# yu-changqian/TorchSeg

Hardware: AMD Instinct MI355X
Metric: training images/sec (1024x1024) BiSeNet-R18 (higher is better)
Workload: dtype bf16

## Files before the change

### torchseg_amd/csrc/clshead.hip

```cpp
#include "tsg_mfma.h"
#include "tsg_dispatch.h"

namespace tsg {

constexpr int CH_MAXN = 32;
constexpr int CH_MAXC = 256;

struct ChGeom { int64_t B, HW, P; int C, N; };

template <int KS>
__global__ __launch_bounds__(256) void cls_fwd_k(const bf16_t* __restrict__ x, const float* __restrict__ w,
                                                 const float* __restrict__ bias, bf16_t* __restrict__ z, ChGeom g) {
  const int lane = threadIdx.x & 63, half = lane >> 5, l31 = lane & 31;
  bf16x8 af[KS];
#pragma unroll
  for (int ks = 0; ks < KS; ++ks) {
    uint32_t pk[4] = {0u, 0u, 0u, 0u};
    if (l31 < g.N) {
      const float* wr = w + (int64_t)l31 * g.C + ks * 16 + half * 8;
      const float4 a = *reinterpret_cast<const float4*>(wr), b = *reinterpret_cast<const float4*>(wr + 4);
      pk[0] = pack2_bf16(a.x, a.y); pk[1] = pack2_bf16(a.z, a.w); pk[2] = pack2_bf16(b.x, b.y); pk[3] = pack2_bf16(b.z, b.w);
    }
    const uint4 v = make_uint4(pk[0], pk[1], pk[2], pk[3]);
    af[ks] = __builtin_bit_cast(bf16x8, v);
  }
  float bs[16];
#pragma unroll
  for (int r = 0; r < 16; ++r) {
    const int n = (r & 3) + 8 * (r >> 2) + 4 * half;
    bs[r] = (bias && n < g.N) ? bias[n] : 0.f;
  }
  const int64_t ngroups = (g.P + 31) / 32;
  const int64_t wid = (int64_t)blockIdx.x * 4 + (threadIdx.x >> 6), nw = (int64_t)gridDim.x * 4;
  for (int64_t grp = wid; grp < ngroups; grp += nw) {
    const int64_t p = grp * 32 + l31;
    const bool ok = p < g.P;
    const bf16_t* xr = x + (ok ? p : g.P - 1) * g.C + half * 8;
    uint4 bv[KS];
#pragma unroll
    for (int ks = 0; ks < KS; ++ks) bv[ks] = *reinterpret_cast<const uint4*>(xr + ks * 16);
    f32x16 acc;
#pragma unroll
    for (int r = 0; r < 16; ++r) acc[r] = bs[r];
#pragma unroll
    for (int ks = 0; ks < KS; ++ks)
      acc = __builtin_amdgcn_mfma_f32_32x32x16_bf16(af[ks], __builtin_bit_cast(bf16x8, bv[ks]), acc, 0, 0, 0);
    if (ok) {
      const int64_t b = p / g.HW, hw = p - b * g.HW;
      bf16_t* zb = z + b * g.N * g.HW + hw;
#pragma unroll
      for (int r = 0; r < 16; ++r) {
        const int n = (r & 3) + 8 * (r >> 2) + 4 * half;
        if (n < g.N) zb[(int64_t)n * g.HW] = f32_to_bf16(acc[r]);
      }
    }
  }
}

constexpr int CH_RUN = 8;

__device__ __forceinline__ float ch_px(uint2 v, int j) {
  const uint32_t word = j < 2 ? v.x : v.y;
  return (j & 1) ? __uint_as_float(word & 0xffff0000u) : __uint_as_float(word << 16);
}

template <int CT>
__global__ __launch_bounds__(256) void cls_dgrad_k(const bf16_t* __restrict__ dz, const float* __restrict__ w,
                                                   bf16_t* __restrict__ dx, ChGeom g) {
  const int lane = threadIdx.x & 63, half = lane >> 5, l31 = lane & 31;
  bf16x8 bw[CT][2];
#pragma unroll
  for (int ct = 0; ct < CT; ++ct)
#pragma unroll
    for (int ks = 0; ks < 2; ++ks) {
      float f[8];
#pragma unroll
      for (int e = 0; e < 8; ++e) {
        const int n = 16 * ks + 8 * half + e;
        f[e] = n < g.N ? w[(int64_t)n * g.C + ct * 32 + l31] : 0.f;
      }
      const uint4 v = make_uint4(pack2_bf16(f[0], f[1]), pack2_bf16(f[2], f[3]), pack2_bf16(f[4], f[5]), pack2_bf16(f[6], f[7]));
      bw[ct][ks] = __builtin_bit_cast(bf16x8, v);
    }
  const int64_t ngroups = (g.P + 31) / 32;
  const int64_t wid = (int64_t)blockIdx.x * 4 + (threadIdx.x >> 6), nw = (int64_t)gridDim.x * 4;
  const bool even = (lane & 1) == 0;
  for (int64_t grp = wid; grp < ngroups; grp += nw) {
    const int64_t p = grp * 32 + l31;
    const bool ok = p < g.P;
    const int64_t pc = ok ? p : g.P - 1, b = pc / g.HW, hw = pc - b * g.HW;
    const bf16_t* zb = dz + b * g.N * g.HW + hw;
    bf16x8 az[2];
#pragma unroll
    for (int ks = 0; ks < 2; ++ks) {
      uint32_t h[8];
#pragma unroll
      for (int e = 0; e < 8; ++e) {
        const int n = 16 * ks + 8 * half + e;
        h[e] = (ok && n < g.N) ? (uint32_t)zb[(int64_t)n * g.HW] : 0u;
      }
      const uint4 v = make_uint4(h[0] | (h[1] << 16), h[2] | (h[3] << 16), h[4] | (h[5] << 16), h[6] | (h[7] << 16));
      az[ks] = __builtin_bit_cast(bf16x8, v);
    }
#pragma unroll
    for (int ct = 0; ct < CT; ++ct) {
      f32x16 acc;
#pragma unroll
      for (int r = 0; r < 16; ++r) acc[r] = 0.f;
      acc = __builtin_amdgcn_mfma_f32_32x32x16_bf16(az[0], bw[ct][0], acc, 0, 0, 0);
      acc = __builtin_amdgcn_mfma_f32_32x32x16_bf16(az[1], bw[ct][1], acc, 0, 0, 0);
#pragma unroll
      for (int q = 0; q < 8; ++q) {
        const int ra = 2 * q, rb = 2 * q + 1;
        const float got = __shfl_xor(even ? acc[rb] : acc[ra], 1, 64);
        const int r = even ? ra : rb;
        const int64_t pr = grp * 32 + (r & 3) + 8 * (r >> 2) + 4 * half;
        const uint32_t word = even ? pack2_bf16(acc[ra], got) : pack2_bf16(got, acc[rb]);
        if (pr < g.P) *reinterpret_cast<uint32_t*>(dx + pr * g.C + ct * 32 + (l31 & ~1)) = word;
      }
    }
  }
}

template <int CT>
__global__ __launch_bounds__(256) void cls_wgrad_k(const bf16_t* __restrict__ dz, const bf16_t* __restrict__ x,
                                                   float* __restrict__ part, ChGeom g) {
  __shared__ float img[CT * 32 * 32];
  const int lane = threadIdx.x & 63, half = lane >> 5, l31 = lane & 31, wave = threadIdx.x >> 6;
  f32x16 acc[CT];
#pragma unroll
  for (int ct = 0; ct < CT; ++ct)
#pragma unroll
    for (int r = 0; r < 16; ++r) acc[ct][r] = 0.f;
  const int64_t nsteps = g.P / 16;
  const int64_t wid = (int64_t)blockIdx.x * 4 + wave, nw = (int64_t)gridDim.x * 4;
  for (int64_t st = wid; st < nsteps; st += nw) {
    const int64_t p0 = st * 16 + 8 * half, b = p0 / g.HW, hw = p0 - b * g.HW;
    uint4 av = make_uint4(0u, 0u, 0u, 0u);
    if (l31 < g.N) av = *reinterpret_cast<const uint4*>(dz + (b * g.N + l31) * g.HW + hw);
    const bf16_t* xr = x + p0 * g.C + l31;
#pragma unroll
    for (int ct = 0; ct < CT; ++ct) {
      uint32_t h[8];
#pragma unroll
      for (int e = 0; e < 8; ++e) h[e] = (uint32_t)xr[(int64_t)e * g.C + ct * 32];
      const uint4 bv = make_uint4(h[0] | (h[1] << 16), h[2] | (h[3] << 16), h[4] | (h[5] << 16), h[6] | (h[7] << 16));
      acc[ct] = __builtin_amdgcn_mfma_f32_32x32x16_bf16(__builtin_bit_cast(bf16x8, av), __builtin_bit_cast(bf16x8, bv), acc[ct], 0, 0, 0);
    }
  }
  for (int wv = 0; wv < 4; ++wv) {
    if (wave == wv) {
#pragma unroll
      for (int ct = 0; ct < CT; ++ct)
#pragma unroll
        for (int r = 0; r < 16; ++r) {
          float* q = img + (ct * 32 + (r & 3) + 8 * (r >> 2) + 4 * half) * 32 + l31;
          *q = (wv == 0 ? 0.f : *q) + acc[ct][r];
        }
    }
    __syncthreads();
  }
  for (int i = threadIdx.x; i < CT * 32 * 32; i += 256) {
    const int ct = i / 1024, n = (i / 32) % 32, c = i % 32;
    if (n < g.N) part[((int64_t)blockIdx.x * g.N + n) * g.C + ct * 32 + c] = img[i];
  }
}

__global__ __launch_bounds__(256) void cls_dbias_k(const bf16_t* __restrict__ dz, float* __restrict__ part_b, ChGeom g) {
  __shared__ float smr[2 * 4];
  const int n = blockIdx.x;
  const int64_t b = blockIdx.y;
  const bf16_t* zp = dz + (b * g.N + n) * g.HW;
  float a = 0.f, dummy = 0.f;
  for (int64_t i = (int64_t)threadIdx.x * CH_RUN; i < g.HW; i += 256 * CH_RUN) {
    const uint4 v = *reinterpret_cast<const uint4*>(zp + i);
    const uint2 lo = make_uint2(v.x, v.y), hi = make_uint2(v.z, v.w);
#pragma unroll
    for (int j = 0; j < 4; ++j) a += ch_px(lo, j) + ch_px(hi, j);
  }
  block_sum2(a, dummy, smr);
  if (threadIdx.x == 0) part_b[b * g.N + n] = a;
}

__global__ __launch_bounds__(256) void cls_wgrad_fold(const float* __restrict__ part, const float* __restrict__ part_b, int nblk,
                                                      int nblk_b, int64_t nw, int N, float* __restrict__ dw,
                                                      float* __restrict__ db) {
  __shared__ double sm[4][64];
  const int col = threadIdx.x & 63, grp = threadIdx.x >> 6;
  const int64_t i = (int64_t)blockIdx.x * 64 + col;
  const bool bias_blk = blockIdx.x == gridDim.x - 1;
  const float* src = bias_blk ? part_b : part;
  const int64_t n_out = bias_blk ? N : nw, idx = bias_blk ? col : i;
  const int nb = bias_blk ? nblk_b : nblk;
  const int per = (nb + 3) / 4, b0 = grp * per, b1 = b0 + per < nb ? b0 + per : nb;
  double t = 0.0;
  if (idx < n_out) {
    for (int b = b0; b < b1; b += 8) {
      float v[8];
#pragma unroll
      for (int u = 0; u < 8; ++u) v[u] = b + u < b1 ? src[(int64_t)(b + u) * n_out + idx] : 0.f;
#pragma unroll
      for (int u = 0; u < 8; ++u) t += (double)v[u];
    }
  }
  sm[grp][col] = t;
  __syncthreads();
  if (grp == 0 && idx < n_out) {
    const double tot = (sm[0][col] + sm[1][col]) + (sm[2][col] + sm[3][col]);
    if (bias_blk) { if (db) db[idx] = (float)tot; }
    else dw[idx] = (float)tot;
  }
}

static int ch_geom(ChGeom* g, int64_t B, int64_t HW, int C, int N) {
  if (B <= 0 || HW <= 0 || C <= 0 || N <= 0 || N > CH_MAXN || C > CH_MAXC || C % 32 || C > 256 || (C & (C - 1)) || HW % 16) return TSG_E_SHAPE;
  if (B * HW > 0x3fffffffffLL / C) return TSG_E_SHAPE;
  g->B = B; g->HW = HW; g->P = B * HW; g->C = C; g->N = N;
  return 0;
}

constexpr int CH_WBLOCKS = 256;

}

using namespace tsg;

extern "C" {

int tsg_cls_head_supported(int dtype, int Cin, int n_classes, int64_t HW) {
  ChGeom g;
  return dtype == TSG_BF16 && ch_geom(&g, 1, HW, Cin, n_classes) == 0;
}

int tsg_cls_head_fwd(const void* x, const float* w, const float* bias, void* z, int64_t B, int64_t HW, int Cin, int n_classes,
                     void* stream) {
  if (!x || !w || !z) return TSG_E_NULL;
  ChGeom g;
  int e = ch_geom(&g, B, HW, Cin, n_classes);
  if (e) return e;
  if (!aligned16(x) || !aligned16(w)) return TSG_E_ALIGN;
  const int64_t ngroups = (g.P + 31) / 32;
  int64_t blocks = (ngroups + 3) / 4;
  if (blocks > 2048) blocks = 2048;
  hipStream_t st = (hipStream_t)stream;
  return with_int<1, 2, 4, 8, 16>(Cin / 16, [&](auto ks) {
    hipLaunchKernelGGL((cls_fwd_k<ks()>), dim3((unsigned)blocks), dim3(256), 0, st, (const bf16_t*)x, w, bias, (bf16_t*)z, g);
    TSG_CHECK_LAUNCH();
    return 0;
  });
}

int tsg_cls_head_dgrad(const void* dz, const float* w, void* dx, int64_t B, int64_t HW, int Cin, int n_classes, void* stream) {
  if (!dz || !w || !dx) return TSG_E_NULL;
  ChGeom g;
  int e = ch_geom(&g, B, HW, Cin, n_classes);
  if (e) return e;
  if (!aligned16(dz) || !aligned16(dx)) return TSG_E_ALIGN;
  const int64_t ngroups = (g.P + 31) / 32;
  int64_t blocks = (ngroups + 3) / 4;
  if (blocks > 1024) blocks = 1024;
  hipStream_t st = (hipStream_t)stream;
  return with_int<1, 2, 4, 8>(Cin / 32, [&](auto ct) {
    hipLaunchKernelGGL((cls_dgrad_k<ct()>), dim3((unsigned)blocks), dim3(256), 0, st, (const bf16_t*)dz, w, (bf16_t*)dx, g);
    TSG_CHECK_LAUNCH();
    return 0;
  });
}

size_t tsg_cls_head_wgrad_ws_bytes(int64_t B, int Cin, int n_classes) {
  if (B <= 0 || Cin <= 0 || n_classes <= 0) return 0;
  return ((size_t)CH_WBLOCKS * n_classes * Cin + (size_t)B * n_classes) * sizeof(float);
}

int tsg_cls_head_wgrad(const void* dz, const void* x, float* dw, float* dbias, int64_t B, int64_t HW, int Cin, int n_classes,
                       void* ws, size_t ws_bytes, void* stream) {
  if (!dz || !x || !dw || !ws) return TSG_E_NULL;
  ChGeom g;
  int e = ch_geom(&g, B, HW, Cin, n_classes);
  if (e) return e;
  if (B > 65535 || ws_bytes < tsg_cls_head_wgrad_ws_bytes(B, Cin, n_classes)) return B > 65535 ? TSG_E_SHAPE : TSG_E_WS;
  if (!aligned16(dz) || !aligned16(x) || !aligned16(ws)) return TSG_E_ALIGN;
  int64_t blocks = (g.P / 16 + 3) / 4;
  if (blocks > CH_WBLOCKS) blocks = CH_WBLOCKS;
  float* part = (float*)ws;
  float* part_b = part + (size_t)CH_WBLOCKS * n_classes * Cin;
  hipStream_t st = (hipStream_t)stream;
  e = with_int<1, 2, 4, 8>(Cin / 32, [&](auto ct) {
    hipLaunchKernelGGL((cls_wgrad_k<ct()>), dim3((unsigned)blocks), dim3(256), 0, st, (const bf16_t*)dz, (const bf16_t*)x, part, g);
    TSG_CHECK_LAUNCH();
    return 0;
  });
  if (e) return e;
  if (dbias) {
    hipLaunchKernelGGL(cls_dbias_k, dim3((unsigned)n_classes, (unsigned)B), dim3(256), 0, st, (const bf16_t*)dz, part_b, g);
    TSG_CHECK_LAUNCH();
  }
  const int64_t nw = (int64_t)n_classes * Cin;
  hipLaunchKernelGGL(cls_wgrad_fold, dim3((unsigned)((nw + 63) / 64 + 1)), dim3(256), 0, st, part, part_b, (int)blocks, (int)B, nw,
                     n_classes, dw, dbias);
  TSG_CHECK_LAUNCH();
  return 0;
}

}
```

### torchseg_amd/csrc/upsample.hip

```cpp
#include "tsg_dispatch.h"
#include "tsg_resample.h"

namespace tsg {

constexpr int kT = 256;

template <typename T, int V> struct OutVec;
template <> struct OutVec<float, 4> : Vec<float> {};
template <> struct OutVec<bf16_t, 8> : Vec<bf16_t> {};
template <typename T> struct OutVec<T, 1> {
  float v[1];
  __device__ __forceinline__ void load(const T* p) { v[0] = ld1<T>(p); }
  __device__ __forceinline__ void store(T* p) const { st1<T>(p, v[0]); }
};

template <typename T> __device__ __forceinline__ float round_as(float v);
template <> __device__ __forceinline__ float round_as<float>(float v) { return v; }
template <> __device__ __forceinline__ float round_as<bf16_t>(float v) { return bf16_to_f32(f32_to_bf16(v)); }

enum { kAddNone = 0, kAddOut = 1, kAddSrc = 2 };

template <typename T, int V, int ADD, int RB>
__global__ __launch_bounds__(kT) void up_fwd(const T* __restrict__ x, const T* __restrict__ add,
                                             T* __restrict__ y, int64_t NC, int IH, int IW, int OH,
                                             int OW, float sy, float sx) {
  const int vpr = OW / V;
  const int bands = (OH + RB - 1) / RB;
  const int64_t total = NC * bands * (int64_t)vpr;
  for (int64_t i = (int64_t)blockIdx.x * kT + threadIdx.x; i < total; i += (int64_t)gridDim.x * kT) {
    const int vx = (int)(i % vpr);
    const int64_t t = i / vpr;
    const int band = (int)(t % bands);
    const int64_t nc = t / bands;
    int x0[V], x1[V];
    float lx[V];
#pragma unroll
    for (int j = 0; j < V; ++j) src_index(sx, vx * V + j, IW, x0[j], x1[j], lx[j]);
    const T* src = x + nc * IH * (int64_t)IW;
    const T* src2 = ADD == kAddSrc ? add + nc * IH * (int64_t)IW : nullptr;
    auto tap = [&](int64_t off) -> float {
      return ADD == kAddSrc ? round_as<T>(ld1<T>(src + off) + ld1<T>(src2 + off)) : ld1<T>(src + off);
    };
    float h0[V], h1[V];
    int cy0 = -1, cy1 = -1;
    const int oy_end = (band + 1) * RB < OH ? (band + 1) * RB : OH;
    for (int oy = band * RB; oy < oy_end; ++oy) {
      int y0, y1; float ly;
      src_index(sy, oy, IH, y0, y1, ly);
      if (y0 != cy0) {
        if (y0 == cy1) {
#pragma unroll
          for (int j = 0; j < V; ++j) h0[j] = h1[j];
        } else {
          const int64_t r = (int64_t)y0 * IW;
#pragma unroll
          for (int j = 0; j < V; ++j) h0[j] = (1.f - lx[j]) * tap(r + x0[j]) + lx[j] * tap(r + x1[j]);
        }
        cy0 = y0;
        cy1 = -1;
      }
      if (y1 != cy1) {
        if (y1 == cy0) {
#pragma unroll
          for (int j = 0; j < V; ++j) h1[j] = h0[j];
        } else {
          const int64_t r = (int64_t)y1 * IW;
#pragma unroll
          for (int j = 0; j < V; ++j) h1[j] = (1.f - lx[j]) * tap(r + x0[j]) + lx[j] * tap(r + x1[j]);
        }
        cy1 = y1;
      }
      const float hy = 1.f - ly;
      const int64_t ooff = (nc * OH + oy) * (int64_t)OW + (int64_t)vx * V;
      OutVec<T, V> o, a;
      if (ADD == kAddOut) a.load(add + ooff);
#pragma unroll
      for (int j = 0; j < V; ++j) {
        float v = hy * h0[j] + ly * h1[j];
        if (ADD == kAddOut) v += a.v[j];
        o.v[j] = v;
      }
      o.store(y + ooff);
    }
  }
}

template <typename T, int MAXF>
__global__ __launch_bounds__(kT) void up_bwd(const T* __restrict__ dy, T* __restrict__ dx,
                                             int64_t NC, int IH, int IW, int OH, int OW, float sy,
                                             float sx) {
  const int64_t total = NC * IH * (int64_t)IW;
  for (int64_t i = (int64_t)blockIdx.x * kT + threadIdx.x; i < total; i += (int64_t)gridDim.x * kT) {
    const int ix = (int)(i % IW);
    const int64_t row = i / IW;
    const int iy = (int)(row % IH);
    const int64_t nc = row / IH;
    int xlo, xhi, ylo, yhi;
    footprint(sx, ix, OW, xlo, xhi);
    footprint(sy, iy, OH, ylo, yhi);
    float acc = 0.f;
    const T* base = dy + nc * OH * (int64_t)OW;
    if (MAXF > 0) {
      float wx[MAXF > 0 ? MAXF : 1];
#pragma unroll
      for (int j = 0; j < MAXF; ++j) wx[j] = (xlo + j <= xhi) ? tap_weight(sx, xlo + j, IW, ix) : 0.f;
      for (int oy = ylo; oy <= yhi; ++oy) {
        const float wy = tap_weight(sy, oy, IH, iy);
        if (wy != 0.f) {
          const T* r = base + (int64_t)oy * OW + xlo;
          float racc = 0.f;
#pragma unroll
          for (int j = 0; j < MAXF; ++j)
            if (xlo + j <= xhi) racc += wx[j] * ld1<T>(r + j);
          acc += wy * racc;
        }
      }
    } else {
      for (int oy = ylo; oy <= yhi; ++oy) {
        const float wy = tap_weight(sy, oy, IH, iy);
        if (wy != 0.f) {
          const T* r = base + (int64_t)oy * OW;
          float racc = 0.f;
          for (int ox = xlo; ox <= xhi; ++ox) racc += tap_weight(sx, ox, IW, ix) * ld1<T>(r + ox);
          acc += wy * racc;
        }
      }
    }
    st1<T>(dx + i, acc);
  }
}

template <typename T, int V, int MAXF>
__global__ void up_bwd_tiled(const T* __restrict__ dy, T* __restrict__ dx, int IH, int IW, int OH,
                             int OW, int RB, float sy, float sx) {
  extern __shared__ __attribute__((aligned(16))) float vrow[];
  const int nthreads = blockDim.x;
  const int tid = threadIdx.x;
  const int vpr = OW / V;
  const int bands = (IH + RB - 1) / RB;
  const int band = blockIdx.x % bands;
  const int64_t nc = blockIdx.x / bands;
  const int r0 = band * RB;
  const int r1 = (r0 + RB < IH) ? r0 + RB : IH;
  const T* src = dy + nc * OH * (int64_t)OW;
  for (int i = tid; i < (r1 - r0) * OW; i += nthreads) vrow[i] = 0.f;
  __syncthreads();
  int oy_lo = 0, oy_hi = OH - 1;
  if (sy > 0.f) {
    const float inv = 1.f / sy;
    int l = (int)ceilf((float)(r0 - 1) * inv) - 1;
    int h = (int)floorf((float)r1 * inv) + 1;
    oy_lo = l < 0 ? 0 : l;
    oy_hi = h > OH - 1 ? OH - 1 : h;
  }
  if (tid < vpr) {
    float accA[V], accB[V];
#pragma unroll
    for (int j = 0; j < V; ++j) { accA[j] = 0.f; accB[j] = 0.f; }
    int cur = -2;
    auto flush = [&](int row, const float (&acc)[V]) {
      if (row >= r0 && row < r1) {
        float* d = vrow + (row - r0) * OW + tid * V;
#pragma unroll
        for (int j = 0; j < V; ++j) d[j] = acc[j];
      }
    };
    auto absorb = [&](int oy, const OutVec<T, V>& g) {
      int y0, y1; float ly;
      src_index(sy, oy, IH, y0, y1, ly);
      if (y0 < r0 - 1 || y0 > r1 - 1) return;
      if (y0 != cur) {
        if (cur >= 0) {
          flush(cur, accA);
          if (y0 == cur + 1) {
#pragma unroll
            for (int j = 0; j < V; ++j) { accA[j] = accB[j]; accB[j] = 0.f; }
          } else {
            flush(cur + 1, accB);
#pragma unroll
            for (int j = 0; j < V; ++j) { accA[j] = 0.f; accB[j] = 0.f; }
          }
        }
        cur = y0;
      }
      const float hy = 1.f - ly;
      if (y1 == y0) {
#pragma unroll
        for (int j = 0; j < V; ++j) accA[j] += hy * g.v[j] + ly * g.v[j];
      } else {
#pragma unroll
        for (int j = 0; j < V; ++j) { accA[j] += hy * g.v[j]; accB[j] += ly * g.v[j]; }
      }
    };
    constexpr int U = 8;
    int oy = oy_lo;
    for (; oy + U - 1 <= oy_hi; oy += U) {
      OutVec<T, V> g[U];
#pragma unroll
      for (int u = 0; u < U; ++u) g[u].load(src + (int64_t)(oy + u) * OW + tid * V);
#pragma unroll
      for (int u = 0; u < U; ++u) absorb(oy + u, g[u]);
    }
    for (; oy <= oy_hi; ++oy) {
      OutVec<T, V> g;
      g.load(src + (int64_t)oy * OW + tid * V);
      absorb(oy, g);
    }
    if (cur >= 0) { flush(cur, accA); flush(cur + 1, accB); }
  }
  __syncthreads();
  for (int ix = tid; ix < IW; ix += nthreads) {
    int xlo, xhi;
    footprint(sx, ix, OW, xlo, xhi);
    float wx[MAXF];
#pragma unroll
    for (int j = 0; j < MAXF; ++j) wx[j] = (xlo + j <= xhi) ? tap_weight(sx, xlo + j, IW, ix) : 0.f;
    for (int r = r0; r < r1; ++r) {
      const float* v = vrow + (r - r0) * OW + xlo;
      float acc = 0.f;
#pragma unroll
      for (int j = 0; j < MAXF; ++j)
        if (xlo + j <= xhi) acc += wx[j] * v[j];
      st1<T>(dx + (nc * IH + r) * (int64_t)IW + ix, acc);
    }
  }
}

template <typename T, int V, int ADD>
__global__ __launch_bounds__(kT) void up_fwd_nhwc(const T* __restrict__ x, const T* __restrict__ add,
                                                  T* __restrict__ y, int64_t N, int C, int IH, int IW,
                                                  int OH, int OW, float sy, float sx) {
  const int G = C / V;
  const int64_t total = N * OH * (int64_t)OW * G;
  for (int64_t i = (int64_t)blockIdx.x * kT + threadIdx.x; i < total; i += (int64_t)gridDim.x * kT) {
    const int g = (int)(i % G);
    int64_t t = i / G;
    const int ox = (int)(t % OW); t /= OW;
    const int oy = (int)(t % OH);
    const int64_t n = t / OH;
    int y0, y1, x0, x1; float ly, lx;
    src_index(sy, oy, IH, y0, y1, ly);
    src_index(sx, ox, IW, x0, x1, lx);
    const float hy = 1.f - ly, hx = 1.f - lx;
    const T* b = x + n * IH * (int64_t)IW * C + g * V;
    OutVec<T, V> p00, p01, p10, p11, o, a;
    p00.load(b + ((int64_t)y0 * IW + x0) * C);
    p01.load(b + ((int64_t)y0 * IW + x1) * C);
    p10.load(b + ((int64_t)y1 * IW + x0) * C);
    p11.load(b + ((int64_t)y1 * IW + x1) * C);
    if (ADD == kAddOut) a.load(add + i * V);
    if (ADD == kAddSrc) {
      const T* b2 = add + n * IH * (int64_t)IW * C + g * V;
      OutVec<T, V> q00, q01, q10, q11;
      q00.load(b2 + ((int64_t)y0 * IW + x0) * C);
      q01.load(b2 + ((int64_t)y0 * IW + x1) * C);
      q10.load(b2 + ((int64_t)y1 * IW + x0) * C);
      q11.load(b2 + ((int64_t)y1 * IW + x1) * C);
#pragma unroll
      for (int j = 0; j < V; ++j) {
        p00.v[j] = round_as<T>(p00.v[j] + q00.v[j]); p01.v[j] = round_as<T>(p01.v[j] + q01.v[j]);
        p10.v[j] = round_as<T>(p10.v[j] + q10.v[j]); p11.v[j] = round_as<T>(p11.v[j] + q11.v[j]);
      }
    }
#pragma unroll
    for (int j = 0; j < V; ++j) {
      float v = hy * (hx * p00.v[j] + lx * p01.v[j]) + ly * (hx * p10.v[j] + lx * p11.v[j]);
      if (ADD == kAddOut) v += a.v[j];
      o.v[j] = v;
    }
    o.store(y + i * V);
  }
}

template <typename T, int V>
__global__ __launch_bounds__(kT) void up_bwd_nhwc(const T* __restrict__ dy, T* __restrict__ dx,
                                                  int64_t N, int C, int IH, int IW, int OH, int OW,
                                                  float sy, float sx) {
  const int G = C / V;
  const int64_t total = N * IH * (int64_t)IW * G;
  for (int64_t i = (int64_t)blockIdx.x * kT + threadIdx.x; i < total; i += (int64_t)gridDim.x * kT) {
    const int g = (int)(i % G);
    int64_t t = i / G;
    const int ix = (int)(t % IW); t /= IW;
    const int iy = (int)(t % IH);
    const int64_t n = t / IH;
    int xlo, xhi, ylo, yhi;
    footprint(sx, ix, OW, xlo, xhi);
    footprint(sy, iy, OH, ylo, yhi);
    float acc[V];
#pragma unroll
    for (int j = 0; j < V; ++j) acc[j] = 0.f;
    const T* b = dy + n * OH * (int64_t)OW * C + g * V;
    for (int oy = ylo; oy <= yhi; ++oy) {
      const float wy = tap_weight(sy, oy, IH, iy);
      if (wy == 0.f) continue;
      for (int ox = xlo; ox <= xhi; ++ox) {
        const float w = wy * tap_weight(sx, ox, IW, ix);
        if (w != 0.f) {
          OutVec<T, V> p;
          p.load(b + ((int64_t)oy * OW + ox) * C);
#pragma unroll
          for (int j = 0; j < V; ++j) acc[j] += w * p.v[j];
        }
      }
    }
    OutVec<T, V> o;
#pragma unroll
    for (int j = 0; j < V; ++j) o.v[j] = acc[j];
    o.store(dx + i * V);
  }
}

template <typename T, int V>
__global__ __launch_bounds__(256) void up_bwd_nhwc_split(const T* __restrict__ dy, T* __restrict__ dx, int64_t N, int C,
                                                         int IH, int IW, int OH, int OW, float sy, float sx, int gpb) {
  __shared__ float red[256 * V];
  const int G = C / V, RS = 256 / gpb;
  const int tid = threadIdx.x, gl = tid % gpb, rs = tid / gpb;
  const int g = blockIdx.y * gpb + gl;
  int64_t t = blockIdx.x;
  const int ix = (int)(t % IW); t /= IW;
  const int iy = (int)(t % IH);
  const int64_t n = t / IH;
  int xlo, xhi, ylo, yhi;
  footprint(sx, ix, OW, xlo, xhi);
  footprint(sy, iy, OH, ylo, yhi);
  float acc[V];
#pragma unroll
  for (int j = 0; j < V; ++j) acc[j] = 0.f;
  if (rs < RS && g < G) {
    const T* b = dy + n * OH * (int64_t)OW * C + g * V;
    for (int oy = ylo + rs; oy <= yhi; oy += RS) {
      const float wy = tap_weight(sy, oy, IH, iy);
      if (wy == 0.f) continue;
      for (int ox = xlo; ox <= xhi; ++ox) {
        const float w = wy * tap_weight(sx, ox, IW, ix);
        if (w != 0.f) {
          OutVec<T, V> p;
          p.load(b + ((int64_t)oy * OW + ox) * C);
#pragma unroll
          for (int j = 0; j < V; ++j) acc[j] += w * p.v[j];
        }
      }
    }
  }
#pragma unroll
  for (int j = 0; j < V; ++j) red[tid * V + j] = acc[j];
  __syncthreads();
  if (rs == 0 && g < G) {
    OutVec<T, V> o;
#pragma unroll
    for (int j = 0; j < V; ++j) {
      float s = 0.f;
      for (int q = 0; q < RS; ++q) s += red[(q * gpb + gl) * V + j];
      o.v[j] = s;
    }
    o.store(dx + (blockIdx.x * (int64_t)G + g) * V);
  }
}

template <int EB>
__global__ __launch_bounds__(kT) void nearest_fwd(const void* __restrict__ x, void* __restrict__ y,
                                                  int64_t NC, int IH, int IW, int OH, int OW,
                                                  float sy, float sx) {
  typedef typename std::conditional<EB == 1, uint8_t,
          typename std::conditional<EB == 2, uint16_t,
          typename std::conditional<EB == 4, uint32_t, uint64_t>::type>::type>::type E;
  const int64_t total = NC * OH * (int64_t)OW;
  for (int64_t i = (int64_t)blockIdx.x * kT + threadIdx.x; i < total; i += (int64_t)gridDim.x * kT) {
    const int ox = (int)(i % OW);
    const int64_t row = i / OW;
    const int oy = (int)(row % OH);
    const int64_t nc = row / OH;
    int iy = (int)floorf((float)oy * sy); if (iy > IH - 1) iy = IH - 1;
    int ix = (int)floorf((float)ox * sx); if (ix > IW - 1) ix = IW - 1;
    ((E*)y)[i] = ((const E*)x)[(nc * IH + iy) * IW + ix];
  }
}

static int grid_for(int64_t work) {
  int64_t g = (work + kT - 1) / kT;
  if (g > 8192) g = 8192;
  if (g < 1) g = 1;
  return (int)g;
}

}

using namespace tsg;

template <typename T, bool ACC>
__global__ __launch_bounds__(kT) void resize_hp_k(const T* __restrict__ x, float* __restrict__ y, int64_t NC, int IH,
                                                  int IW, int OH, int OW) {
  const double sy = 1.0 / ((double)OH / (double)IH), sx = 1.0 / ((double)OW / (double)IW);
  const int64_t total = NC * OH * (int64_t)OW;
  for (int64_t i = (int64_t)blockIdx.x * kT + threadIdx.x; i < total; i += (int64_t)gridDim.x * kT) {
    const int ox = (int)(i % OW);
    const int64_t t = i / OW;
    const int oy = (int)(t % OH);
    const int64_t nc = t / OH;
    int y0, y1, x0, x1; float wy, wx;
    hp_index(oy, sy, IH, y0, y1, wy);
    hp_index(ox, sx, IW, x0, x1, wx);
    const T* p = x + nc * IH * (int64_t)IW;
    const float a = ld1<T>(p + (int64_t)y0 * IW + x0), b = ld1<T>(p + (int64_t)y0 * IW + x1);
    const float c = ld1<T>(p + (int64_t)y1 * IW + x0), d = ld1<T>(p + (int64_t)y1 * IW + x1);
    const float v = (1.f - wy) * ((1.f - wx) * a + wx * b) + wy * ((1.f - wx) * c + wx * d);
    y[i] = ACC ? y[i] + v : v;
  }
}

extern "C" {

static int up_fwd_launch(const void* x, const void* add, int add_mode, void* y, int dtype, int64_t NC,
                         int IH, int IW, int OH, int OW, void* stream) {
  if (!x || !y || (add_mode != kAddNone && !add)) return TSG_E_NULL;
  if (dtype != TSG_F32 && dtype != TSG_BF16) return TSG_E_DTYPE;
  if (NC <= 0 || IH <= 0 || IW <= 0 || OH <= 0 || OW <= 0) return TSG_E_SHAPE;
  hipStream_t st = (hipStream_t)stream;
  const float sy = ac_scale(IH, OH), sx = ac_scale(IW, OW);
  const int native = native_vec(dtype);
  const bool vec = (OW % native == 0) && aligned16(y) && (add_mode != kAddOut || aligned16(add));
  const int V = vec ? native : 1;
  const int grid = grid_for(NC * ((OH + 15) / 16) * (int64_t)(OW / V));
  return with_elem_vec(dtype, vec, [&](auto t, auto v) { return with_int<kAddOut, kAddSrc, kAddNone>(add_mode, [&](auto a) {
    typedef typename decltype(t)::type T;
    hipLaunchKernelGGL((up_fwd<T, v(), a(), 16>), dim3(grid), dim3(kT), 0, st, (const T*)x, (const T*)add, (T*)y, NC, IH, IW,
                       OH, OW, sy, sx);
    TSG_CHECK_LAUNCH();
    return 0;
  }); });
}

int tsg_upsample_bilinear_ac_fwd(const void* x, const void* add, void* y, int dtype, int64_t NC,
                                 int IH, int IW, int OH, int OW, void* stream) {
  return up_fwd_launch(x, add, add ? kAddOut : kAddNone, y, dtype, NC, IH, IW, OH, OW, stream);
}

int tsg_upsample_bilinear_ac_presum_fwd(const void* x, const void* x2, void* y, int dtype, int64_t NC,
                                        int IH, int IW, int OH, int OW, void* stream) {
  return up_fwd_launch(x, x2, kAddSrc, y, dtype, NC, IH, IW, OH, OW, stream);
}

int tsg_upsample_bilinear_ac_bwd(const void* dy, void* dx, int dtype, int64_t NC, int IH, int IW,
                                 int OH, int OW, void* stream) {
  if (!dy || !dx) return TSG_E_NULL;
  if (dtype != TSG_F32 && dtype != TSG_BF16) return TSG_E_DTYPE;
  if (NC <= 0 || IH <= 0 || IW <= 0 || OH <= 0 || OW <= 0) return TSG_E_SHAPE;
  hipStream_t st = (hipStream_t)stream;
  const float sy = ac_scale(IH, OH), sx = ac_scale(IW, OW);
  int need = sx > 0.f ? (int)floorf(2.f / sx) + 4 : OW;
  const int maxf = need <= 9 ? 9 : need <= 21 ? 21 : need <= 37 ? 37 : 0;
  const int native = native_vec(dtype);
  if (need <= 37 && OW % native == 0 && OW / native <= 1024 && OW >= IW && aligned16(dy)) {
    int threads = ((OW / native + 63) / 64) * 64;
    if (threads < 128) threads = 128;
    int RB = 8;
    while (RB > 1 && (size_t)RB * OW * sizeof(float) > 48 * 1024) RB >>= 1;
    if ((size_t)RB * OW * sizeof(float) <= 64 * 1024) {
      const int bands = (IH + RB - 1) / RB;
      const int64_t blocks = NC * bands;
      if (blocks <= 0x7fffffffLL) {
        const size_t sh = (size_t)RB * OW * sizeof(float);
        return with_elem(dtype, [&](auto t) { return with_int<9, 21, 37>(maxf, [&](auto f) {
          typedef typename decltype(t)::type T;
          hipLaunchKernelGGL((up_bwd_tiled<T, Vec<T>::N, f()>), dim3((unsigned)blocks), dim3(threads), sh, st, (const T*)dy,
                             (T*)dx, IH, IW, OH, OW, RB, sy, sx);
          TSG_CHECK_LAUNCH();
          return 0;
        }); });
      }
    }
  }
  const int grid = grid_for(NC * IH * (int64_t)IW);
  return with_elem(dtype, [&](auto t) { return with_int<9, 21, 37, 0>(maxf, [&](auto f) {
    typedef typename decltype(t)::type T;
    hipLaunchKernelGGL((up_bwd<T, f()>), dim3(grid), dim3(kT), 0, st, (const T*)dy, (T*)dx, NC, IH, IW, OH, OW, sy, sx);
    TSG_CHECK_LAUNCH();
    return 0;
  }); });
}

static int up_fwd_nhwc_launch(const void* x, const void* add, int add_mode, void* y, int dtype, int64_t N,
                              int C, int IH, int IW, int OH, int OW, void* stream) {
  if (!x || !y || (add_mode != kAddNone && !add)) return TSG_E_NULL;
  if (dtype != TSG_F32 && dtype != TSG_BF16) return TSG_E_DTYPE;
  const int V = native_vec(dtype);
  if (N <= 0 || C <= 0 || C % V || IH <= 0 || IW <= 0 || OH <= 0 || OW <= 0) return TSG_E_SHAPE;
  if (!aligned16(x) || !aligned16(y) || (add && !aligned16(add))) return TSG_E_ALIGN;
  hipStream_t st = (hipStream_t)stream;
  const float sy = ac_scale(IH, OH), sx = ac_scale(IW, OW);
  const int grid = grid_for(N * OH * (int64_t)OW * (C / V));
  return with_elem(dtype, [&](auto t) { return with_int<kAddOut, kAddSrc, kAddNone>(add_mode, [&](auto a) {
    typedef typename decltype(t)::type T;
    hipLaunchKernelGGL((up_fwd_nhwc<T, Vec<T>::N, a()>), dim3(grid), dim3(kT), 0, st, (const T*)x, (const T*)add, (T*)y, N, C,
                       IH, IW, OH, OW, sy, sx);
    TSG_CHECK_LAUNCH();
    return 0;
  }); });
}

int tsg_upsample_bilinear_ac_nhwc_fwd(const void* x, const void* add, void* y, int dtype, int64_t N,
                                      int C, int IH, int IW, int OH, int OW, void* stream) {
  return up_fwd_nhwc_launch(x, add, add ? kAddOut : kAddNone, y, dtype, N, C, IH, IW, OH, OW, stream);
}

int tsg_upsample_bilinear_ac_nhwc_presum_fwd(const void* x, const void* x2, void* y, int dtype, int64_t N,
                                             int C, int IH, int IW, int OH, int OW, void* stream) {
  return up_fwd_nhwc_launch(x, x2, kAddSrc, y, dtype, N, C, IH, IW, OH, OW, stream);
}

int tsg_upsample_bilinear_ac_nhwc_bwd(const void* dy, void* dx, int dtype, int64_t N, int C, int IH,
                                      int IW, int OH, int OW, void* stream) {
  if (!dy || !dx) return TSG_E_NULL;
  if (dtype != TSG_F32 && dtype != TSG_BF16) return TSG_E_DTYPE;
  const int V = native_vec(dtype);
  if (N <= 0 || C <= 0 || C % V || IH <= 0 || IW <= 0 || OH <= 0 || OW <= 0) return TSG_E_SHAPE;
  if (!aligned16(dy) || !aligned16(dx)) return TSG_E_ALIGN;
  hipStream_t st = (hipStream_t)stream;
  const float sy = ac_scale(IH, OH), sx = ac_scale(IW, OW);
  const int G = C / V;
  if (N * IH * (int64_t)IW * G < 65536 && OH >= 8 * IH && N * IH * (int64_t)IW <= 0x7fffffffLL) {
    int gpb = 256;
    while (gpb > G) gpb >>= 1;
    if (gpb < 1) gpb = 1;
    while (gpb > 8 && N * IH * (int64_t)IW * ((G + gpb - 1) / gpb) < 512) gpb >>= 1;
    const dim3 grid2((unsigned)(N * IH * IW), (unsigned)((G + gpb - 1) / gpb));
    return with_elem(dtype, [&](auto t) {
      typedef typename decltype(t)::type T;
      hipLaunchKernelGGL((up_bwd_nhwc_split<T, Vec<T>::N>), grid2, dim3(256), 0, st, (const T*)dy, (T*)dx, N, C, IH, IW, OH, OW,
                         sy, sx, gpb);
      TSG_CHECK_LAUNCH();
      return 0;
    });
  }
  const int grid = grid_for(N * IH * (int64_t)IW * (C / V));
  return with_elem(dtype, [&](auto t) {
    typedef typename decltype(t)::type T;
    hipLaunchKernelGGL((up_bwd_nhwc<T, Vec<T>::N>), dim3(grid), dim3(kT), 0, st, (const T*)dy, (T*)dx, N, C, IH, IW, OH, OW, sy, sx);
    TSG_CHECK_LAUNCH();
    return 0;
  });
}

int tsg_upsample_nearest_fwd(const void* x, void* y, int elem_bytes, int64_t NC, int IH, int IW,
                             int OH, int OW, void* stream) {
  if (!x || !y) return TSG_E_NULL;
  if (NC <= 0 || IH <= 0 || IW <= 0 || OH <= 0 || OW <= 0) return TSG_E_SHAPE;
  hipStream_t st = (hipStream_t)stream;
  const float sy = (float)IH / (float)OH, sx = (float)IW / (float)OW;
  const int grid = grid_for(NC * OH * (int64_t)OW);
#define GO(EB) hipLaunchKernelGGL((nearest_fwd<EB>), dim3(grid), dim3(kT), 0, st, x, y, NC, IH, IW, OH, OW, sy, sx)
  switch (elem_bytes) {
    case 1: GO(1); break;
    case 2: GO(2); break;
    case 4: GO(4); break;
    case 8: GO(8); break;
    default: return TSG_E_DTYPE;
  }
#undef GO
  TSG_CHECK_LAUNCH();
  return 0;
}

int tsg_resize_bilinear_hp(const void* x, float* y, int dtype, int64_t NC, int IH, int IW, int OH, int OW,
                           int accumulate, void* stream) {
  if (!x || !y) return TSG_E_NULL;
  if (dtype != TSG_F32 && dtype != TSG_BF16) return TSG_E_DTYPE;
  if (NC <= 0 || IH <= 0 || IW <= 0 || OH <= 0 || OW <= 0) return TSG_E_SHAPE;
  hipStream_t st = (hipStream_t)stream;
  const int grid = grid_for(NC * OH * (int64_t)OW);
  return with_elem(dtype, [&](auto t) { return with_flag(accumulate != 0, [&](auto acc) {
    typedef typename decltype(t)::type T;
    hipLaunchKernelGGL((resize_hp_k<T, acc()>), dim3(grid), dim3(kT), 0, st, (const T*)x, y, NC, IH, IW, OH, OW);
    TSG_CHECK_LAUNCH();
    return 0;
  }); });
}

}
```

Baseline: 1336.

## Add LDS-staged streaming class-head kernels and row-strip bilinear upsample

Result: no change. 1344 (median of 6 runs) (+0.6%).

```diff
diff --git a/torchseg_amd/csrc/clshead.hip b/torchseg_amd/csrc/clshead.hip
--- a/torchseg_amd/csrc/clshead.hip
+++ b/torchseg_amd/csrc/clshead.hip
@@ -53,6 +53,87 @@
         const int n = (r & 3) + 8 * (r >> 2) + 4 * half;
         if (n < g.N) zb[(int64_t)n * g.HW] = f32_to_bf16(acc[r]);
       }
+    }
+  }
+}
+
+typedef u32x4 __attribute__((may_alias)) lds_u32x4;
+__device__ __forceinline__ void wave_lds_sync() {
+  __builtin_amdgcn_fence(__ATOMIC_RELEASE, "wavefront");
+  __builtin_amdgcn_wave_barrier();
+  __builtin_amdgcn_fence(__ATOMIC_ACQUIRE, "wavefront");
+}
+__device__ __forceinline__ u32x4 zero_u32x4() { const u32x4 z = {0u, 0u, 0u, 0u}; return z; }
+
+template <int KS>
+__global__ __launch_bounds__(KS == 16 ? 128 : 256) void cls_fwd_stream_k(const bf16_t* __restrict__ x,
+                                                                         const float* __restrict__ w,
+                                                                         const float* __restrict__ bias,
+                                                                         bf16_t* __restrict__ z, ChGeom g) {
+  constexpr int W = KS == 16 ? 2 : 4;
+  constexpr int C = KS * 16, ROW = C / 8 + 1;
+  __shared__ uint4 tile[W * 32 * ROW];
+  const int lane = threadIdx.x & 63, half = lane >> 5, l31 = lane & 31, wave = threadIdx.x >> 6;
+  uint4* my = tile + wave * 32 * ROW;
+  bf16x8 af[KS];
+#pragma unroll
+  for (int ks = 0; ks < KS; ++ks) {
+    uint32_t pk[4] = {0u, 0u, 0u, 0u};
+    if (l31 < g.N) {
+      const float* wr = w + (int64_t)l31 * C + ks * 16 + half * 8;
+      const float4 a = *reinterpret_cast<const float4*>(wr), b = *reinterpret_cast<const float4*>(wr + 4);
+      pk[0] = pack2_bf16(a.x, a.y); pk[1] = pack2_bf16(a.z, a.w); pk[2] = pack2_bf16(b.x, b.y); pk[3] = pack2_bf16(b.z, b.w);
+    }
+    const uint4 v = make_uint4(pk[0], pk[1], pk[2], pk[3]);
+    af[ks] = __builtin_bit_cast(bf16x8, v);
+  }
+  float bs[16];
+#pragma unroll
+  for (int r = 0; r < 16; ++r) {
+    const int n = (r & 3) + 8 * (r >> 2) + 4 * half;
+    bs[r] = (bias && n < g.N) ? bias[n] : 0.f;
+  }
+  const int64_t ngroups = (g.P + 31) / 32;
+  const bool even = (lane & 1) == 0;
+  auto fetch = [&](int64_t grp, uint4 (&bv)[KS]) {
+    const int64_t left = (g.P - grp * 32) * (C / 8);
+    const uint4* src = reinterpret_cast<const uint4*>(x) + grp * 32 * (C / 8) + lane;
+#pragma unroll
+    for (int i = 0; i < KS; ++i) bv[i] = i * 64 + lane < left ? src[i * 64] : make_uint4(0u, 0u, 0u, 0u);
+  };
+  const int64_t wid = (int64_t)blockIdx.x * W + wave, nw = (int64_t)gridDim.x * W;
+  uint4 bv[KS];
+  if (wid < ngroups) fetch(wid, bv);
+  for (int64_t grp = wid; grp < ngroups; grp += nw) {
+#pragma unroll
+    for (int i = 0; i < KS; ++i) {
+      const int j = i * 64 + lane;
+      my[(j / (C / 8)) * ROW + j % (C / 8)] = bv[i];
+    }
+    wave_lds_sync();
+    if (grp + nw < ngroups) fetch(grp + nw, bv);
+    f32x16 acc;
+#pragma unroll
+    for (int r = 0; r < 16; ++r) acc[r] = bs[r];
+#pragma unroll
+    for (int ks = 0; ks < KS; ++ks) {
+      const uint4 fr = my[l31 * ROW + 2 * ks + half];
+      acc = __builtin_amdgcn_mfma_f32_32x32x16_bf16(af[ks], __builtin_bit_cast(bf16x8, fr), acc, 0, 0, 0);
+    }
+    wave_lds_sync();
+    const int64_t p = grp * 32 + (l31 & ~1);
+    const bool ok = p < g.P;
+    const int64_t pc = ok ? p : 0, b = pc / g.HW, hw = pc - b * g.HW;
+    bf16_t* zb = z + b * g.N * g.HW + hw;
+#pragma unroll
+    for (int q = 0; q < 8; ++q) {
+      const int ra = 2 * q, rb = 2 * q + 1;
+      const float got = __shfl_xor(even ? acc[rb] : acc[ra], 1, 64);
+      const int r = even ? ra : rb;
+      const int n = (r & 3) + 8 * (r >> 2) + 4 * half;
+      const uint32_t word = even ? ((uint32_t)f32_to_bf16(acc[ra]) | ((uint32_t)f32_to_bf16(got) << 16))
+                                 : ((uint32_t)f32_to_bf16(got) | ((uint32_t)f32_to_bf16(acc[rb]) << 16));
+      if (ok && n < g.N) *reinterpret_cast<uint32_t*>(zb + (int64_t)n * g.HW) = word;
     }
   }
 }
@@ -123,6 +204,92 @@
 }
 
 template <int CT>
+__global__ __launch_bounds__(256) void cls_dgrad_stream_k(const bf16_t* __restrict__ dz, const float* __restrict__ w,
+                                                          bf16_t* __restrict__ dx, ChGeom g) {
+  constexpr int CP = CT >= 2 ? 2 : 1;
+  constexpr int OROW = CP == 2 ? 192 : 64;
+  constexpr int WB = 2048 + 32 * OROW;
+  __shared__ __attribute__((aligned(16))) unsigned char lds[4 * WB];
+  const int lane = threadIdx.x & 63, half = lane >> 5, l31 = lane & 31, sub = (lane >> 4) & 1, i16 = lane & 15;
+  unsigned char* zt = lds + (threadIdx.x >> 6) * WB;
+  unsigned char* ot = zt + 2048;
+  const lds_v4i16* zfr = (const lds_v4i16*)(zt + (8 * half + (i16 >> 2)) * 64 + (16 * sub + 4 * (i16 & 3)) * 2);
+  bf16x8 bw[CT][2];
+#pragma unroll
+  for (int ct = 0; ct < CT; ++ct)
+#pragma unroll
+    for (int ks = 0; ks < 2; ++ks) {
+      float f[8];
+#pragma unroll
+      for (int e = 0; e < 8; ++e) {
+        const int n = 16 * ks + 8 * half + e;
+        f[e] = n < g.N ? w[(int64_t)n * g.C + ct * 32 + l31] : 0.f;
+      }
+      const uint4 v = make_uint4(pack2_bf16(f[0], f[1]), pack2_bf16(f[2], f[3]), pack2_bf16(f[4], f[5]), pack2_bf16(f[6], f[7]));
+      bw[ct][ks] = __builtin_bit_cast(bf16x8, v);
+    }
+  const int64_t ngroups = (g.P + 31) / 32;
+  const int64_t wid = (int64_t)blockIdx.x * 4 + (threadIdx.x >> 6), nw = (int64_t)gridDim.x * 4;
+  const bool even = (lane & 1) == 0;
+  auto fetch = [&](int64_t grp, u32x4 (&zv)[2]) {
+#pragma unroll
+    for (int i = 0; i < 2; ++i) {
+      const int q = lane + 64 * i, n = q >> 2;
+      const int64_t p0 = grp * 32 + 8 * (q & 3);
+      zv[i] = zero_u32x4();
+      if (n < g.N && p0 < g.P) {
+        const int64_t b = p0 / g.HW, hw = p0 - b * g.HW;
+        zv[i] = *reinterpret_cast<const u32x4*>(dz + (b * g.N + n) * g.HW + hw);
+      }
+    }
+  };
+  u32x4 zv[2];
+  if (wid < ngroups) fetch(wid, zv);
+  for (int64_t grp = wid; grp < ngroups; grp += nw) {
+#pragma unroll
+    for (int i = 0; i < 2; ++i) *reinterpret_cast<lds_u32x4*>(zt + (lane + 64 * i) * 16) = zv[i];
+    wave_lds_sync();
+    union { v4i16 q[2]; bf16x8 v; } az[2];
+#pragma unroll
+    for (int ks = 0; ks < 2; ++ks) {
+      az[ks].q[0] = __builtin_amdgcn_ds_read_tr16_b64_v4i16((lds_v4i16*)(zfr + ks * 128));
+      az[ks].q[1] = __builtin_amdgcn_ds_read_tr16_b64_v4i16((lds_v4i16*)(zfr + ks * 128 + 32));
+    }
+    if (grp + nw < ngroups) fetch(grp + nw, zv);
+#pragma unroll
+    for (int cp = 0; cp < CT / CP; ++cp) {
+#pragma unroll
+      for (int c2 = 0; c2 < CP; ++c2) {
+        const int ct = cp * CP + c2;
+        f32x16 acc;
+#pragma unroll
+        for (int r = 0; r < 16; ++r) acc[r] = 0.f;
+        acc = __builtin_amdgcn_mfma_f32_32x32x16_bf16(az[0].v, bw[ct][0], acc, 0, 0, 0);
+        acc = __builtin_amdgcn_mfma_f32_32x32x16_bf16(az[1].v, bw[ct][1], acc, 0, 0, 0);
+#pragma unroll
+        for (int q = 0; q < 8; ++q) {
+          const int ra = 2 * q, rb = 2 * q + 1;
+          const float got = __shfl_xor(even ? acc[rb] : acc[ra], 1, 64);
+          const int r = even ? ra : rb;
+          const int row = (r & 3) + 8 * (r >> 2) + 4 * half;
+          const uint32_t word = even ? pack2_bf16(acc[ra], got) : pack2_bf16(got, acc[rb]);
+          *reinterpret_cast<lds_u32*>(ot + row * OROW + (c2 * 32 + (l31 & ~1)) * 2) = word;
+        }
+      }
+      wave_lds_sync();
+#pragma unroll
+      for (int i = 0; i < 2 * CP; ++i) {
+        const int j = i * 64 + lane, px = j / (CP * 4), cc = j % (CP * 4);
+        const u32x4 v = *reinterpret_cast<const lds_u32x4*>(ot + px * OROW + cc * 16);
+        const int64_t pr = grp * 32 + px;
+        if (pr < g.P) *reinterpret_cast<u32x4*>(dx + pr * g.C + cp * CP * 32 + cc * 8) = v;
+      }
+      wave_lds_sync();
+    }
+  }
+}
+
+template <int CT>
 __global__ __launch_bounds__(256) void cls_wgrad_k(const bf16_t* __restrict__ dz, const bf16_t* __restrict__ x,
                                                    float* __restrict__ part, ChGeom g) {
   __shared__ float img[CT * 32 * 32];
@@ -148,6 +315,83 @@
       acc[ct] = __builtin_amdgcn_mfma_f32_32x32x16_bf16(__builtin_bit_cast(bf16x8, av), __builtin_bit_cast(bf16x8, bv), acc[ct], 0, 0, 0);
     }
   }
+  for (int wv = 0; wv < 4; ++wv) {
+    if (wave == wv) {
+#pragma unroll
+      for (int ct = 0; ct < CT; ++ct)
+#pragma unroll
+        for (int r = 0; r < 16; ++r) {
+          float* q = img + (ct * 32 + (r & 3) + 8 * (r >> 2) + 4 * half) * 32 + l31;
+          *q = (wv == 0 ? 0.f : *q) + acc[ct][r];
+        }
+    }
+    __syncthreads();
+  }
+  for (int i = threadIdx.x; i < CT * 32 * 32; i += 256) {
+    const int ct = i / 1024, n = (i / 32) % 32, c = i % 32;
+    if (n < g.N) part[((int64_t)blockIdx.x * g.N + n) * g.C + ct * 32 + c] = img[i];
+  }
+}
+
+constexpr int CW_D = 3;
+
+template <int CT>
+__global__ __launch_bounds__(256) void cls_wgrad_stream_k(const bf16_t* __restrict__ dz, const bf16_t* __restrict__ x,
+                                                          float* __restrict__ part, ChGeom g) {
+  constexpr int C = CT * 32;
+  constexpr int XROW = (2 * C) % 256 == 64 ? 2 * C : 2 * C + 64;
+  constexpr int WB = 16 * XROW;
+  constexpr int IMGB = CT * 32 * 32 * 4;
+  __shared__ __attribute__((aligned(16))) unsigned char lds[4 * WB > IMGB ? 4 * WB : IMGB];
+  float* img = reinterpret_cast<float*>(lds);
+  const int lane = threadIdx.x & 63, half = lane >> 5, l31 = lane & 31, wave = threadIdx.x >> 6;
+  const int sub = (lane >> 4) & 1, i16 = lane & 15;
+  unsigned char* xt = lds + wave * WB;
+  const lds_v4i16* xfr = (const lds_v4i16*)(xt + (8 * half + (i16 >> 2)) * XROW + (16 * sub + 4 * (i16 & 3)) * 2);
+  f32x16 acc[CT];
+#pragma unroll
+  for (int ct = 0; ct < CT; ++ct)
+#pragma unroll
+    for (int r = 0; r < 16; ++r) acc[ct][r] = 0.f;
+  const int64_t nsteps = g.P / 16;
+  const int64_t wid = (int64_t)blockIdx.x * 4 + wave, nw = (int64_t)gridDim.x * 4;
+  u32x4 xv[CW_D][CT], av[CW_D];
+  auto fetch = [&](int d, int64_t st) {
+    const int64_t p0 = st * 16 + 8 * half, b = p0 / g.HW, hw = p0 - b * g.HW;
+    av[d] = zero_u32x4();
+    if (l31 < g.N) av[d] = *reinterpret_cast<const u32x4*>(dz + (b * g.N + l31) * g.HW + hw);
+    const u32x4* src = reinterpret_cast<const u32x4*>(x + st * 16 * C) + lane;
+#pragma unroll
+    for (int i = 0; i < CT; ++i) xv[d][i] = src[i * 64];
+  };
+#pragma unroll
+  for (int d = 0; d < CW_D; ++d)
+    if (wid + d * nw < nsteps) fetch(d, wid + d * nw);
+  for (int64_t st0 = wid; st0 < nsteps; st0 += CW_D * nw) {
+#pragma unroll
+    for (int d = 0; d < CW_D; ++d) {
+      const int64_t st = st0 + d * nw;
+      if (st < nsteps) {
+#pragma unroll
+        for (int i = 0; i < CT; ++i) {
+          const int j = i * 64 + lane;
+          *reinterpret_cast<lds_u32x4*>(xt + (j / (C / 8)) * XROW + (j % (C / 8)) * 16) = xv[d][i];
+        }
+        const bf16x8 af = __builtin_bit_cast(bf16x8, av[d]);
+        wave_lds_sync();
+        if (st + CW_D * nw < nsteps) fetch(d, st + CW_D * nw);
+#pragma unroll
+        for (int ct = 0; ct < CT; ++ct) {
+          union { v4i16 q[2]; bf16x8 v; } fb;
+          fb.q[0] = __builtin_amdgcn_ds_read_tr16_b64_v4i16((lds_v4i16*)(xfr + ct * 8));
+          fb.q[1] = __builtin_amdgcn_ds_read_tr16_b64_v4i16((lds_v4i16*)(xfr + ct * 8 + XROW / 2));
+          acc[ct] = __builtin_amdgcn_mfma_f32_32x32x16_bf16(af, fb.v, acc[ct], 0, 0, 0);
+        }
+        wave_lds_sync();
+      }
+    }
+  }
+  __syncthreads();
   for (int wv = 0; wv < 4; ++wv) {
     if (wave == wv) {
 #pragma unroll
@@ -221,6 +465,8 @@
 
 constexpr int CH_WBLOCKS = 256;
 
+static bool cls_stream() { return tsg_env_flag("TSG_CLS_STREAM", true); }
+
 }
 
 using namespace tsg;
@@ -243,6 +489,17 @@
   int64_t blocks = (ngroups + 3) / 4;
   if (blocks > 2048) blocks = 2048;
   hipStream_t st = (hipStream_t)stream;
+  if (cls_stream() && Cin >= 64) {
+    const int wpb = Cin == 256 ? 2 : 4;
+    blocks = (ngroups + wpb - 1) / wpb;
+    if (blocks > 512) blocks = 512;
+    return with_int<4, 8, 16>(Cin / 16, [&](auto ks) {
+      hipLaunchKernelGGL((cls_fwd_stream_k<ks()>), dim3((unsigned)blocks), dim3(64 * wpb), 0, st, (const bf16_t*)x, w, bias,
+                         (bf16_t*)z, g);
+      TSG_CHECK_LAUNCH();
+      return 0;
+    });
+  }
   return with_int<1, 2, 4, 8, 16>(Cin / 16, [&](auto ks) {
     hipLaunchKernelGGL((cls_fwd_k<ks()>), dim3((unsigned)blocks), dim3(256), 0, st, (const bf16_t*)x, w, bias, (bf16_t*)z, g);
     TSG_CHECK_LAUNCH();
@@ -260,6 +517,12 @@
   int64_t blocks = (ngroups + 3) / 4;
   if (blocks > 1024) blocks = 1024;
   hipStream_t st = (hipStream_t)stream;
+  if (cls_stream())
+    return with_int<1, 2, 4, 8>(Cin / 32, [&](auto ct) {
+      hipLaunchKernelGGL((cls_dgrad_stream_k<ct()>), dim3((unsigned)blocks), dim3(256), 0, st, (const bf16_t*)dz, w, (bf16_t*)dx, g);
+      TSG_CHECK_LAUNCH();
+      return 0;
+    });
   return with_int<1, 2, 4, 8>(Cin / 32, [&](auto ct) {
     hipLaunchKernelGGL((cls_dgrad_k<ct()>), dim3((unsigned)blocks), dim3(256), 0, st, (const bf16_t*)dz, w, (bf16_t*)dx, g);
     TSG_CHECK_LAUNCH();
@@ -285,8 +548,13 @@
   float* part = (float*)ws;
   float* part_b = part + (size_t)CH_WBLOCKS * n_classes * Cin;
   hipStream_t st = (hipStream_t)stream;
+  const bool streamk = cls_stream();
   e = with_int<1, 2, 4, 8>(Cin / 32, [&](auto ct) {
-    hipLaunchKernelGGL((cls_wgrad_k<ct()>), dim3((unsigned)blocks), dim3(256), 0, st, (const bf16_t*)dz, (const bf16_t*)x, part, g);
+    if (streamk)
+      hipLaunchKernelGGL((cls_wgrad_stream_k<ct()>), dim3((unsigned)blocks), dim3(256), 0, st, (const bf16_t*)dz, (const bf16_t*)x,
+                         part, g);
+    else
+      hipLaunchKernelGGL((cls_wgrad_k<ct()>), dim3((unsigned)blocks), dim3(256), 0, st, (const bf16_t*)dz, (const bf16_t*)x, part, g);
     TSG_CHECK_LAUNCH();
     return 0;
   });
diff --git a/torchseg_amd/csrc/upsample.hip b/torchseg_amd/csrc/upsample.hip
--- a/torchseg_amd/csrc/upsample.hip
+++ b/torchseg_amd/csrc/upsample.hip
@@ -272,6 +272,73 @@
   }
 }
 
+template <typename T, int V, int ADD>
+__global__ __launch_bounds__(kT) void up_fwd_strip(const T* __restrict__ x, const T* __restrict__ add,
+                                                   T* __restrict__ y, int C, int IH, int IW, int OH, int OW,
+                                                   float sy, float sx, int RS) {
+  const int G = C / V, rowv = OW * G;
+  const int idx = blockIdx.x * kT + threadIdx.x;
+  if (idx >= rowv) return;
+  const int ox = idx / G, g = idx - ox * G;
+  const int64_t n = blockIdx.z;
+  int x0, x1; float lx;
+  src_index(sx, ox, IW, x0, x1, lx);
+  const float hx = 1.f - lx;
+  const T* b = x + n * IH * (int64_t)IW * C + g * V;
+  const T* b2 = ADD == kAddSrc ? add + n * IH * (int64_t)IW * C + g * V : nullptr;
+  auto hrow = [&](int yy, float (&h)[V]) {
+    const int64_t o0 = ((int64_t)yy * IW + x0) * C, o1 = ((int64_t)yy * IW + x1) * C;
+    OutVec<T, V> p0, p1;
+    p0.load(b + o0);
+    p1.load(b + o1);
+    if (ADD == kAddSrc) {
+      OutVec<T, V> q0, q1;
+      q0.load(b2 + o0);
+      q1.load(b2 + o1);
+#pragma unroll
+      for (int j = 0; j < V; ++j) { p0.v[j] = round_as<T>(p0.v[j] + q0.v[j]); p1.v[j] = round_as<T>(p1.v[j] + q1.v[j]); }
+    }
+#pragma unroll
+    for (int j = 0; j < V; ++j) h[j] = hx * p0.v[j] + lx * p1.v[j];
+  };
+  float top[V], bot[V];
+  int cy0 = -1, cy1 = -1;
+  const int oy0 = blockIdx.y * RS, oy1 = oy0 + RS < OH ? oy0 + RS : OH;
+  for (int oy = oy0; oy < oy1; ++oy) {
+    int y0, y1; float ly;
+    src_index(sy, oy, IH, y0, y1, ly);
+    if (y0 != cy0) {
+      if (y0 == cy1) {
+#pragma unroll
+        for (int j = 0; j < V; ++j) top[j] = bot[j];
+      } else {
+        hrow(y0, top);
+      }
+      cy0 = y0;
+    }
+    if (y1 != cy1) {
+      if (y1 == cy0) {
+#pragma unroll
+        for (int j = 0; j < V; ++j) bot[j] = top[j];
+      } else {
+        hrow(y1, bot);
+      }
+      cy1 = y1;
+    }
+    const float hy = 1.f - ly;
+    const int64_t ooff = ((n * OH + oy) * (int64_t)rowv + idx) * V;
+    OutVec<T, V> o, a;
+    if (ADD == kAddOut) a.load(add + ooff);
+#pragma unroll
+    for (int j = 0; j < V; ++j) {
+      float v = hy * top[j] + ly * bot[j];
+      if (ADD == kAddOut) v += a.v[j];
+      o.v[j] = v;
+    }
+    o.store(y + ooff);
+  }
+}
+
 template <typename T, int V>
 __global__ __launch_bounds__(kT) void up_bwd_nhwc(const T* __restrict__ dy, T* __restrict__ dx,
                                                   int64_t N, int C, int IH, int IW, int OH, int OW,
@@ -377,6 +444,8 @@
     ((E*)y)[i] = ((const E*)x)[(nc * IH + iy) * IW + ix];
   }
 }
+
+static bool up_strip() { return tsg_env_flag("TSG_UP_STRIP", true); }
 
 static int grid_for(int64_t work) {
   int64_t g = (work + kT - 1) / kT;
@@ -490,6 +559,23 @@
   if (!aligned16(x) || !aligned16(y) || (add && !aligned16(add))) return TSG_E_ALIGN;
   hipStream_t st = (hipStream_t)stream;
   const float sy = ac_scale(IH, OH), sx = ac_scale(IW, OW);
+  const int64_t rowv = (int64_t)OW * (C / V);
+  if (up_strip() && rowv <= 0x3fffffff && N <= 65535) {
+    const int64_t chunks = (rowv + kT - 1) / kT;
+    int RS = 8;
+    while (RS > 2 && N * chunks * ((OH + RS - 1) / RS) < 1024) RS >>= 1;
+    const int64_t strips = (OH + RS - 1) / RS;
+    if (strips <= 65535) {
+      const dim3 grid3((unsigned)chunks, (unsigned)strips, (unsigned)N);
+      return with_elem(dtype, [&](auto t) { return with_int<kAddOut, kAddSrc, kAddNone>(add_mode, [&](auto a) {
+        typedef typename decltype(t)::type T;
+        hipLaunchKernelGGL((up_fwd_strip<T, Vec<T>::N, a()>), grid3, dim3(kT), 0, st, (const T*)x, (const T*)add, (T*)y, C, IH, IW,
+                           OH, OW, sy, sx, RS);
+        TSG_CHECK_LAUNCH();
+        return 0;
+      }); });
+    }
+  }
   const int grid = grid_for(N * OH * (int64_t)OW * (C / V));
   return with_elem(dtype, [&](auto t) { return with_int<kAddOut, kAddSrc, kAddNone>(add_mode, [&](auto a) {
     typedef typename decltype(t)::type T;
```
